# JuanJoZP/cfd-hemodynamic

Measured on AMD Instinct MI355X. Metric: time-steps/sec, dfg_1 ~1M DOF (stabilized_schur), higher is better.
Workload: dtype f64 (fp32 only in the AMG matrix values of the flexible preconditioner and in a read-only copy of the Krylov basis that Gram-Schmidt reads in solves of >= 20 iterations)

## Files before the change

### cfd_hemodynamic_amd/csrc/cfdh_api.cpp

```cpp
#include <algorithm>
#include <cmath>
#include <numeric>

#include <dlfcn.h>

#include "cfdh_internal.hpp"

std::string g_cfdh_last_error;

int cfdh_prepare_assembly(cfdh_ctx *c);

#define ENTER(c)                         \
  do {                                   \
    if (!(c)) return CFDH_E_ARG;         \
    (void)hipSetDevice((c)->device);     \
  } while (0)

extern "C" {

int cfdh_abi_version(void) { return CFDH_ABI_VERSION; }

const char *cfdh_last_error(const cfdh_ctx *c) { return c ? c->err.c_str() : g_cfdh_last_error.c_str(); }

int cfdh_default_options(cfdh_options *o) {
// ... 5 lines not shown
  o->pc_refresh = 0; o->remove_p_mean = 1; o->verbose = 0; o->pc_type = 1; o->cc_smooth_degree = 2;
  o->ksp_guess = getenv("CFDH_KSP_GUESS") ? atoi(getenv("CFDH_KSP_GUESS")) : 4;
  return 0;
}

static int create_ctx(cfdh_ctx **out, int device, int gdim, int etype, int64_t nv, int64_t nv_owned, int64_t nc, const int32_t *cells,
                      const double *coords, int64_t nfacets, const int32_t *facet_cells, const int32_t *facet_local,
                      const int32_t *facet_marker) {
  if (!out) return cfdh_fail(nullptr, CFDH_E_ARG, "null output pointer");
  *out = nullptr;
  if (gdim != 2 && gdim != 3) return cfdh_fail(nullptr, CFDH_E_ARG, "gdim must be 2 (P1 triangles) or 3 (P1 tetrahedra)");
  if (etype < 0 || etype > 3) return cfdh_fail(nullptr, CFDH_E_ARG, "unknown element type %d", etype);
  if (!cells || !coords || (nfacets > 0 && (!facet_cells || !facet_local)))
    return cfdh_fail(nullptr, CFDH_E_ARG, "null mesh array");
  int ndev = 0;
  if (hipGetDeviceCount(&ndev) != hipSuccess || ndev <= 0)
    return cfdh_fail(nullptr, CFDH_E_HIP, "no HIP device available: libcfdh has no CPU fallback");
  if (device < 0 || device >= ndev) return cfdh_fail(nullptr, CFDH_E_ARG, "device %d out of range (%d devices)", device, ndev);
  cfdh_ctx *c = new (std::nothrow) cfdh_ctx();
  if (!c) return cfdh_fail(nullptr, CFDH_E_NOMEM, "out of host memory");
  c->device = device;
  cfdh_default_options(&c->opt);
  { const char *e = getenv("CFDH_NO_GRAPH"); c->use_graph = !(e && e[0] == '1'); }
  if (c->use_graph && (getenv("ROCP_TOOL_LIBRARIES") || dlsym(RTLD_DEFAULT, "rocprofiler_configure"))) {
    int rt = 0;
    const char *ov = getenv("CFDH_GRAPH_UNDER_PROFILER");
    if (!(ov && ov[0] == '1') && hipRuntimeGetVersion(&rt) == hipSuccess && rt >= 70200000) c->use_graph = false;
  }
  memset(&c->last_stats, 0, sizeof c->last_stats);
  int rc = 0;
  do {
    if (hipSetDevice(device) != hipSuccess) { rc = cfdh_fail(nullptr, CFDH_E_HIP, "hipSetDevice(%d) failed", device); break; }
    if (hipStreamCreateWithFlags(&c->stream, hipStreamNonBlocking) != hipSuccess) { rc = cfdh_fail(nullptr, CFDH_E_HIP, "hipStreamCreate failed"); break; }
    rc = gdim == 3 ? k3_upload_quadrature(c) : k_upload_quadrature(c);
    if (rc) break;
    if (etype != 0) {
      rc = gdim == 3 ? kg3_upload_tables(c) : kg_upload_tables(c);
      if (rc) break;
      rc = gdim == 3 ? cfdh_build_mesh_gen3(c, etype, nv, nv_owned, nc, cells, coords, nfacets, facet_cells, facet_local, facet_marker)
                     : cfdh_build_mesh_gen(c, etype, nv, nv_owned, nc, cells, coords, nfacets, facet_cells, facet_local, facet_marker);
      break;
    }
    rc = gdim == 3 ? cfdh_build_mesh3(c, nv, nv_owned, nc, cells, coords, nfacets, facet_cells, facet_local, facet_marker)
                   : cfdh_build_mesh(c, nv, nv_owned, nc, cells, coords, nfacets, facet_cells, facet_local, facet_marker);
  } while (0);
  if (rc) {
// ... 15 lines not shown
                     int64_t nfacets, const int32_t *facet_cells, const int32_t *facet_local, const int32_t *facet_marker) {
  return create_ctx(out, device, gdim, elem, nn, nn, nc, cells, node_coords, nfacets, facet_cells, facet_local, facet_marker);
}

int cfdh_create_elem_part(cfdh_ctx **out, int device, int gdim, int elem, int64_t nn, int64_t nn_owned, int64_t nc, const int32_t *cells,
                          const double *node_coords, int64_t nfacets, const int32_t *facet_cells, const int32_t *facet_local, const int32_t *facet_marker) {
  return create_ctx(out, device, gdim, elem, nn, nn_owned, nc, cells, node_coords, nfacets, facet_cells, facet_local, facet_marker);
}

void cfdh_destroy(cfdh_ctx *c) {
  if (!c) return;
  (void)hipSetDevice(c->device);
  if (c->stream) (void)hipStreamSynchronize(c->stream);
  comm_finalize(c);
  c->hS.clear(); c->hL.clear(); c->hA.clear(); c->hLg.clear();
  for (hipEvent_t e : c->ev_pool) (void)hipEventDestroy(e);
  for (auto &e : c->pc_graphs) for (auto &x : e.exec) if (x) (void)hipGraphExecDestroy(x);
  if (c->h_pinned) (void)hipHostFree(c->h_pinned);
  if (c->h_stage) (void)hipHostFree(c->h_stage);
  if (c->ev_h) (void)hipEventDestroy(c->ev_h);
  if (c->h_big) (void)hipHostFree(c->h_big);
  if (c->h_ring) (void)hipHostFree(c->h_ring);
  for (hipEvent_t e : c->ev_ring) if (e) (void)hipEventDestroy(e);
  hipStream_t s = c->stream;
  delete c;
  if (s) (void)hipStreamDestroy(s);
}

int cfdh_set_params(cfdh_ctx *c, double dt, double rho, double mu, double mu_facet, const double f[3]) {
  ENTER(c);
  if (!(dt > 0) || !(rho > 0) || !(mu > 0)) return cfdh_fail(c, CFDH_E_ARG, "dt, rho, mu must be positive");
  const bool changed = !c->params_set || dt != c->dt || rho != c->rho || mu != c->mu;
  c->dt = dt; c->rho = rho; c->mu = mu; c->muf = mu_facet;
  c->f[0] = f ? f[0] : 0.0; c->f[1] = f ? f[1] : 0.0; c->f[2] = (f && c->dim == 3) ? f[2] : 0.0;
  c->params_set = true;
  if (changed) { c->mom_valid = false; c->pc_valid = false; }
  return 0;
}

int cfdh_set_options(cfdh_ctx *c, const cfdh_options *o) {
  if (!c || !o) return CFDH_E_ARG;
  if (o->ksp_restart < 1 || o->ksp_restart > 1000 || o->cheb_degree < 1 || o->cc_smooth_degree < 1 || !(o->cheb_ratio > 1) || o->amg_smooth_degree < 1 ||
      !(o->amg_smooth_ratio > 1) || o->amg_max_coarse < 8 || o->amg_max_coarse > 4000 || o->ksp_guess < 0 || o->ksp_guess > 8)
    return cfdh_fail(c, CFDH_E_ARG, "option out of range");
  const bool pc_changed = o->amg_theta != c->opt.amg_theta || o->amg_max_coarse != c->opt.amg_max_coarse ||
                          o->amg_smooth_ratio != c->opt.amg_smooth_ratio || o->pc_type != c->opt.pc_type ||
                          o->amg_smooth_degree != c->opt.amg_smooth_degree ||
                          o->schur_full != c->opt.schur_full;
// ... 682 lines not shown
```

### cfd_hemodynamic_amd/csrc/cfdh_internal.hpp

```cpp
#pragma once
#include <hip/hip_runtime.h>

#include <cstdint>
#include <cstdio>
#include <cstring>
#include <string>
#include <vector>

#include "cfdh.h"

#ifndef CFDH_MAX_INC
#define CFDH_MAX_INC 256
#endif
#ifndef CFDH_MAX_BV
#define CFDH_MAX_BV 192
#endif
#ifndef CFDH_MAX_BC
#define CFDH_MAX_BC 192
#endif
#ifndef CFDH_MAX_ROWS
#define CFDH_MAX_ROWS 128
#endif

#if defined(__HIPCC__)
// ... 215 lines not shown
  dbuf<double> kV, kZ, kw, kh;
  dbuf<float> kV32;
  bool krylov_fp32_ok = true;
  int guess_last_its[4] = {0, 0, 0, 0};
  dbuf<double> ky;

  dbuf<double> dinvA;
  double lmaxA = 0;
  dbuf<double> pu0, pu1, pu2, pr, pp0, pp1;
  dbuf<double> prand;
  dbuf<double> cheb_coef;
  struct PcGraph { const double *r; double *z; hipGraphExec_t exec[6]; };
  std::vector<PcGraph> pc_graphs;
  bool pc_graph_valid = false, capturing = false, use_graph = true;
  AmgHier hS;
  AmgHier hL;
  AmgHier hA;
  AmgLevel Hlev;
  dbuf<double> ccMl;
  dbuf<unsigned char> ccPbc;
  double cc_alpha = 0, cc_beta = 0;
  int up0_rows = 0;
  struct Epilogue { bool on = false, done = false; double alpha = 0, beta = 0; const double *zH = nullptr, *r = nullptr; const unsigned char *pbc = nullptr; double *out = nullptr; } epi;
  std::vector<double> h_Lval, h_Ml;
  dbuf<double> d_Lval, d_Ml;
  dbuf<double> amg_rand;
  double ms_pc_build_dev = 0;
  long long bc_version = 0;
  int gp_n = 0;
  CsrHost gp_L;
  bool gp_singular = false, gp_dirty = false;
  AmgHier hLg;
  dbuf<int> gp_l2g;
  dbuf<double> gp_rhs, gp_sol;
  bool ras = false;
  std::vector<int> h_gid;
  std::vector<int> h_g2l;
  dbuf<double> ras_b, ras_x;
  struct RasPlan {
    bool ready = false;
    int maxlen = 0;
    int nent = 0;
    dbuf<int> gptr, gcol, gsrc;
    dbuf<double> gval;
  } rasp;
  struct DistL0 {
// ... 97 lines not shown
int kg_assemble(cfdh_ctx *c, const double *xstate, int mode);
int kg_functional_partials(cfdh_ctx *c, int kind, int marker, int nb);
int kg_wss(cfdh_ctx *c, double *out);

int kg3_upload_tables(cfdh_ctx *c);
int cfdh_build_mesh_gen3(cfdh_ctx *c, int etype, int64_t nv, int64_t nv_owned, int64_t nc, const int32_t *cells, const double *coords, int64_t nfac,
                         const int32_t *fcell, const int32_t *flocal, const int32_t *fmarker);
int cfdh_gen3_element_stiffness(const cfdh_ctx *c, const int32_t *v, const double *X, double *K);
int cfdh_facet_nodes3(const cfdh_ctx *c, int f, int out[8]);
int kg3_assemble(cfdh_ctx *c, const double *xstate, int mode);
int kg3_functional_partials(cfdh_ctx *c, int kind, int marker, int nb);
int kg3_wss(cfdh_ctx *c, double *out);

void prof_begin(cfdh_ctx *c, int kind);
void prof_end(cfdh_ctx *c, int kind);
void prof_flush(cfdh_ctx *c);

int k_upload_quadrature(cfdh_ctx *c);
int k_halo_pack(cfdh_ctx *c, const double *vec);
int v_pointwise_mult(cfdh_ctx *c, int n, const double *a, const double *b, double *out);
int k_moments(cfdh_ctx *c);
int k_assemble(cfdh_ctx *c, const double *xstate, int mode);
int k_spmv_full(cfdh_ctx *c, const double *x, double *y);
int k_spmv_full_multi(cfdh_ctx *c, const double *X, double *Y, int ld, int nvec);
int k_spmv_block(cfdh_ctx *c, int blk, const double *x, double *y, const double *b, double alpha);
int k_spmv_block_ghost(cfdh_ctx *c, int blk, const double *xv, double *y, const double *b);
int k_extract_diag(cfdh_ctx *c);
int k_cheb_a00(cfdh_ctx *c, const double *b, double *x);
int k_cheb_a00_coeffs(cfdh_ctx *c);
int k_csr_spmv(cfdh_ctx *c, const CsrDev &A, const double *x, double *y, int mode, const double *b);
int k_csr_spmv_ncol(cfdh_ctx *c, const CsrDev &A, const double *x, double *y, int mode, const double *b, int ncol);
int k_amg_vcycle(cfdh_ctx *c, AmgHier &H, const double *b, double *x);
int k_level_smooth(cfdh_ctx *c, AmgLevel *L, const double *b, double *x, int degree);
bool k_cc_cheb2_scale(cfdh_ctx *c, AmgLevel *L, const double *b, double *x, const double *ml, double *y);
int k_cc_scale(cfdh_ctx *c, int n, const double *ml, const double *z, double *y);
int k_dl0_down(cfdh_ctx *c, const double *halo_vec);
int k_dl0_up(cfdh_ctx *c, double *out);
int k_ext_pack(cfdh_ctx *c, const double *vec, double *out);
int k_scatter_global(cfdh_ctx *c, int n, const int *l2g, const double *loc, double *glob);
int k_gather_global(cfdh_ctx *c, int n, const int *l2g, const double *glob, double *loc);
int k_cc_combine(cfdh_ctx *c, int n, double alpha, double beta, const double *t, const double *z, const double *r, const unsigned char *pbc, double *out, double *out2 = nullptr);
int k_nullspace_test(cfdh_ctx *c, double *nrm, double *absnrm);
int k_bc_scatter(cfdh_ctx *c, int n, int ncomp, const int *idx, const unsigned char *flag, const double *val, const double *mult);

int v_copy(cfdh_ctx *c, int n, const double *x, double *y);
int v_zero(cfdh_ctx *c, int n, double *y);
// ... 39 lines not shown
```

### cfd_hemodynamic_amd/csrc/cfdh_kernels.hip

```cpp
#include <hip/hip_runtime.h>

#include <cmath>

#include "cfdh_internal.hpp"
#include "cfdh_quad_tri.h"

#define TPB 256
#define NTLOAD(p) __builtin_nontemporal_load(p)

__constant__ double d_qw[CFDH_NQ];
__constant__ double d_ql[CFDH_NQ][3];

int k_upload_quadrature(cfdh_ctx *c) {
  HIPCHK(c, hipMemcpyToSymbol(HIP_SYMBOL(d_qw), CFDH_QW, sizeof(CFDH_QW)));
  HIPCHK(c, hipMemcpyToSymbol(HIP_SYMBOL(d_ql), CFDH_QL, sizeof(CFDH_QL)));
  return 0;
}

void prof_begin(cfdh_ctx *c, int kind) {
  if (!c->prof_on || c->capturing) return;
  if (c->ev_next + 2 > c->ev_pool.size()) {
    for (int i = 0; i < 64; i++) { hipEvent_t e; if (hipEventCreate(&e) != hipSuccess) return; c->ev_pool.push_back(e); }
  }
  cfdh_ctx::EvRec r;
// ... 731 lines not shown
  if (row < nvo) {
    const int ks = vptr[row], ke = vptr[row + 1];
    if (l == 0) bb = *(const double2 *)(bvec + 2 * (size_t)row);
    const int k0 = ks + l, k1 = k0 + 4;
    const bool h0 = k0 < ke, h1 = k1 < ke;
    const int q0 = h0 ? k0 : ks, q1 = h1 ? k1 : ks;
    const int w0 = vcol[q0], w1 = vcol[q1];
    const double2 c0 = *(const double2 *)(A + 2 * (size_t)q0), c1 = *(const double2 *)(A + 2 * (size_t)q1);
    const double x0 = (h0 && w0 < nvo) ? x[w0] : 0.0, x1 = (h1 && w1 < nvo) ? x[w1] : 0.0;
    a0 = c0.x * x0 + c1.x * x1;
    a1 = c0.y * x0 + c1.y * x1;
    for (int k = k1 + 4; k < ke; k += 4) {
      const int w = vcol[k];
      if (w >= nvo) continue;
      const double xp = x[w];
      const double2 cc = *(const double2 *)(A + 2 * (size_t)k);
      a0 += cc.x * xp; a1 += cc.y * xp;
    }
  }
  a0 = quad_sum(a0); a1 = quad_sum(a1);
  if (row < nvo && l == 0) *(double2 *)(y + 2 * (size_t)row) = make_double2(bb.x - a0, bb.y - a1);
}

template <int GB>
__global__ __launch_bounds__(TPB) void spmv_blk_ghost_kernel(int nvo, const int *__restrict__ vptr, const int *__restrict__ vcol,
                                                             const double *__restrict__ A, const double *__restrict__ xv,
                                                             double *__restrict__ y, const double *__restrict__ bvec) {
  const int gid = blockIdx.x * TPB + threadIdx.x;
  const int row = gid >> 3, l = gid & 7;
  double a0 = 0, a1 = 0;
  if (row < nvo) {
    const int ks = vptr[row], ke = vptr[row + 1];
    for (int k = ks + l; k < ke; k += 8) {
      const int w = vcol[k];
      const double2 cc = *(const double2 *)(A + 2 * (size_t)k);
      if (GB == 2) {
        const double xp = xv[poff(w, nvo)];
        a0 += cc.x * xp; a1 += cc.y * xp;
      } else {
        const int uo = uoff(w, nvo);
        a0 += cc.x * xv[uo] + cc.y * xv[uo + 1];
      }
    }
  }
  a0 = group8_sum(a0);
  if (GB == 2) a1 = group8_sum(a1);
// ... 583 lines not shown
    T gb[2], gc[2];
#pragma unroll
    for (int q = 0; q < 2; q++) {
      if (kb + 8 * q < keB) gb[q] = b[cb[q]];
      if (kc + 8 * q < keC) gc[q] = xc[cc[q]];
    }
#pragma unroll
    for (int q = 0; q < 2; q++) {
      if (kb + 8 * q < keB) a = vfma(vb[q], gb[q], a);
      if (kc + 8 * q < keC) a = vfma(vc[q], gc[q], a);
    }
    for (int k = kb + 16; k < keB; k += 8) a = vfma(vlB[k], b[clB[k]], a);
    for (int k = kc + 16; k < keC; k += 8) a = vfma(vlC[k], xc[clC[k]], a);
  }
  a = g8(a);
  if (row < n && l == 0) x[row] = epbc ? epi_apply(a, row, ea, eb, ezH, er, epbc) : a;
}
template <typename T, bool WIDE>
__global__ __launch_bounds__(TPB) void fused_up_sell_kernel(int n, const int *__restrict__ spB, const int *__restrict__ scB,
                                                            const float *__restrict__ svB, const T *__restrict__ b,
                                                            const int *__restrict__ spC, const int *__restrict__ scC,
                                                            const float *__restrict__ svC, const T *__restrict__ xc,
                                                            T *__restrict__ x, double ea, double eb, const double *__restrict__ ezH,
                                                            const double *__restrict__ er, const unsigned char *__restrict__ epbc) {
  const int row = blockIdx.x * TPB + threadIdx.x;
  if (row >= n) return;
  const int sl = __builtin_amdgcn_readfirstlane(row >> 6), lane = row & 63;
  T a = vzero((const T *)nullptr);
  double e_zh = 0.0, e_r = 0.0;
  unsigned e_f = 0;
  if (epbc) { e_f = epbc[row]; e_zh = ezH[row]; e_r = er[row]; }
  constexpr int MW = sizeof(T) > 8 ? 8 : 10;
  const int pB = spB[sl], wB = (spB[sl + 1] - pB) >> 6;
  int pC = 0, wC = 0;
  if (spC) { pC = spC[sl]; wC = (spC[sl + 1] - pC) >> 6; }
  const int wmax = wB > wC ? wB : wC;
  for (int k0 = 0; k0 < (WIDE ? wmax : 1); k0 += MW) {
    int cB[MW], cC[MW];
    float vB[MW], vC[MW];
#pragma unroll
    for (int k = 0; k < MW; k++) if (k0 + k < wB) { const int p = pB + (k0 + k) * 64 + lane; cB[k] = NTLOAD(scB + p); vB[k] = NTLOAD(svB + p); }
#pragma unroll
    for (int k = 0; k < MW; k++) if (k0 + k < wC) { const int p = pC + (k0 + k) * 64 + lane; cC[k] = NTLOAD(scC + p); vC[k] = NTLOAD(svC + p); }
    T gB[MW], gC[MW];
#pragma unroll
    for (int k = 0; k < MW; k++) if (k0 + k < wB) gB[k] = b[cB[k]];
#pragma unroll
    for (int k = 0; k < MW; k++) if (k0 + k < wC) gC[k] = xc[cC[k]];
#pragma unroll
    for (int k = 0; k < MW; k++) if (k0 + k < wB) a = vfma((double)vB[k], gB[k], a);
#pragma unroll
    for (int k = 0; k < MW; k++) if (k0 + k < wC) a = vfma((double)vC[k], gC[k], a);
  }
  if (!WIDE) {
    for (int k = MW; k < wB; k++) { const int p = pB + k * 64 + lane; a = vfma((double)svB[p], b[scB[p]], a); }
    for (int k = MW; k < wC; k++) { const int p = pC + k * 64 + lane; a = vfma((double)svC[p], xc[scC[p]], a); }
// ... 17 lines not shown
    for (int q = 0; q < 12; q++) { const int j = l + 64 * q; if (j < nc) { dv[q] = Dr[j]; bv[q] = bc[j]; } }
#pragma unroll
    for (int q = 0; q < 12; q++) { const int j = l + 64 * q; if (j < nc) a = vfma((double)dv[q], bv[q], a); }
    for (int j = l + 768; j < nc; j += 64) a = vfma((double)Dr[j], bc[j], a);
  }
  a = wsum(a);
  if (row < n && l == 0) x[row] = a;
}

template <typename VT, typename T>
static void launch_down(cfdh_ctx *c, const CsrDev &G, const VT *val, const T *x, T *y) {
  const long long avg = G.n > 0 ? (G.nnz + G.n - 1) / G.n : 1;
  const int lpr = avg > 96 ? 64 : (avg > 48 ? 32 : (avg > 20 ? 16 : 8));
  dim3 block(TPB), grid((unsigned)(((long long)G.n * lpr + TPB - 1) / TPB));
  if (lpr == 64) hipLaunchKernelGGL((fused_down_kernel<64, VT, T>), grid, block, 0, c->stream, G.n, G.rowptr.p, G.col.p, val, x, y);
  else if (lpr == 32) hipLaunchKernelGGL((fused_down_kernel<32, VT, T>), grid, block, 0, c->stream, G.n, G.rowptr.p, G.col.p, val, x, y);
  else if (lpr == 16) hipLaunchKernelGGL((fused_down_kernel<16, VT, T>), grid, block, 0, c->stream, G.n, G.rowptr.p, G.col.p, val, x, y);
  else hipLaunchKernelGGL((fused_down_kernel<8, VT, T>), grid, block, 0, c->stream, G.n, G.rowptr.p, G.col.p, val, x, y);
}

template <typename T>
static int amg_cycle_fused(cfdh_ctx *c, AmgHier &H, const T *b, T *x, int prof, int l0 = 0) {
  const int nl = (int)H.lev.size();
  for (int l = l0; l + 1 < nl; l++) {
    AmgLevel *L = H.lev[l], *N = H.lev[l + 1];
    const T *src = l == l0 ? b : (const T *)L->b.p;
    if (prof && l == 0) prof_begin(c, prof + 4);
    if (L->fine) launch_down<float, T>(c, L->G, L->G.valf.p, src, (T *)N->b.p);
    else launch_down<double, T>(c, L->G, L->G.val.p, src, (T *)N->b.p);
    if (prof && l == 0) prof_end(c, prof + 4);
  }
  int l = nl - 1;
  {
    AmgLevel *L = H.lev[l];
    const T *bl = l == l0 ? b : (const T *)L->b.p;
    T *xl = l == l0 ? x : (T *)L->x.p;
    if (nl - 2 >= l0 && H.lev[nl - 2]->Dn > 0) {
      AmgLevel *U = H.lev[nl - 2];
      const T *bu = nl - 2 == l0 ? b : (const T *)U->b.p;
      T *xu = nl - 2 == l0 ? x : (T *)U->x.p;
      const int un = (nl - 2 == 0 && c->up0_rows > 0 && c->up0_rows < U->n) ? c->up0_rows : U->n;
      hipLaunchKernelGGL((fused_up_dense_kernel<T>), dim3((unsigned)((64ll * un + TPB - 1) / TPB)), dim3(TPB), 0, c->stream, un,
                         U->Sb.rowptr.p, U->Sb.col.p, U->Sb.val.p, bu, U->D.p, U->Dn, bl, xu);
      l = nl - 3;
    } else {
      if (H.coarse_n > 0)
        hipLaunchKernelGGL((dense_mv_kernel<T>), dim3(H.coarse_n), dim3(64), 0, c->stream, H.coarse_n, H.coarse_inv.p, bl, xl);
      else if (L->sell)
        hipLaunchKernelGGL((fused_up_sell_kernel<T, true>), dim3((unsigned)((L->n + TPB - 1) / TPB)), dim3(TPB), 0, c->stream, L->n,
                           L->Sb.sptr.p, L->Sb.scol.p, L->Sb.sval.p, bl, (const int *)nullptr, (const int *)nullptr,
                           (const float *)nullptr, (const T *)nullptr, xl, 0.0, 0.0, (const double *)nullptr, (const double *)nullptr,
                           (const unsigned char *)nullptr);
      else
        hipLaunchKernelGGL((fused_up_csr_kernel<T>), dim3((unsigned)((8ll * L->n + TPB - 1) / TPB)), dim3(TPB), 0, c->stream, L->n,
                           L->Sb.rowptr.p, L->Sb.col.p, L->Sb.val.p, bl, (const int *)nullptr, (const int *)nullptr,
                           (const double *)nullptr, (const T *)nullptr, xl, 0.0, 0.0, (const double *)nullptr, (const double *)nullptr,
                           (const unsigned char *)nullptr);
      l = nl - 2;
    }
  }
  for (; l >= l0; l--) {
    AmgLevel *L = H.lev[l], *N = H.lev[l + 1];
    const T *bl = l == l0 ? b : (const T *)L->b.p;
    T *xl = l == l0 ? x : (T *)L->x.p;
    const bool epi = l == 0 && c->epi.on && sizeof(T) == sizeof(double);
    const double ea = epi ? c->epi.alpha : 0.0, eb = epi ? c->epi.beta : 0.0;
    const double *ezH = epi ? c->epi.zH : nullptr, *er = epi ? c->epi.r : nullptr;
    const unsigned char *epbc = epi ? c->epi.pbc : nullptr;
    if (epi) { xl = (T *)c->epi.out; c->epi.done = true; }
    const int nrow = (l == 0 && c->up0_rows > 0 && c->up0_rows < L->n) ? c->up0_rows : L->n;
    if (prof && l == 0) prof_begin(c, prof);
    if (L->sell && L->Sb.sell_maxw <= 14 && L->Sc.sell_maxw <= 14)
      hipLaunchKernelGGL((fused_up_sell_kernel<T, false>), dim3((unsigned)((nrow + TPB - 1) / TPB)), dim3(TPB), 0, c->stream, nrow,
                         L->Sb.sptr.p, L->Sb.scol.p, L->Sb.sval.p, bl, L->Sc.sptr.p, L->Sc.scol.p, L->Sc.sval.p, (const T *)N->x.p, xl,
                         ea, eb, ezH, er, epbc);
    else if (L->sell)
      hipLaunchKernelGGL((fused_up_sell_kernel<T, true>), dim3((unsigned)((nrow + TPB - 1) / TPB)), dim3(TPB), 0, c->stream, nrow,
                         L->Sb.sptr.p, L->Sb.scol.p, L->Sb.sval.p, bl, L->Sc.sptr.p, L->Sc.scol.p, L->Sc.sval.p, (const T *)N->x.p, xl,
                         ea, eb, ezH, er, epbc);
    else
      hipLaunchKernelGGL((fused_up_csr_kernel<T>), dim3((unsigned)((8ll * nrow + TPB - 1) / TPB)), dim3(TPB), 0, c->stream, nrow,
                         L->Sb.rowptr.p, L->Sb.col.p, L->Sb.val.p, bl, L->Sc.rowptr.p, L->Sc.col.p, L->Sc.val.p, (const T *)N->x.p, xl,
                         ea, eb, ezH, er, epbc);
    if (prof && l == 0) prof_end(c, prof);
  }
  HIPCHK(c, hipGetLastError());
  return 0;
}

static int amg_cycle_cheb(cfdh_ctx *c, AmgHier &H, size_t lev, const double *b, double *x, bool prof) {
  AmgLevel *L = H.lev[lev];
  if (lev + 1 == H.lev.size()) {
    if (H.coarse_n > 0) {
      hipLaunchKernelGGL((dense_mv_kernel<double>), dim3(H.coarse_n), dim3(64), 0, c->stream, H.coarse_n, H.coarse_inv.p, b, x);
      HIPCHK(c, hipGetLastError());
      return 0;
    }
    return level_cheb(c, L, b, x, true, c->opt.amg_smooth_degree > 2 ? c->opt.amg_smooth_degree : 2, false);
  }
  AmgLevel *N = H.lev[lev + 1];
  const int deg = c->opt.amg_smooth_degree;
  CHK(level_cheb(c, L, b, x, true, deg, prof && lev == 0));
  CHK(k_csr_spmv(c, L->A, x, L->r.p, 1, b));
  CHK(k_csr_spmv(c, L->R, L->r.p, N->b.p, 0, nullptr));
  CHK(amg_cycle_cheb(c, H, lev + 1, N->b.p, N->x.p, prof));
  CHK(k_csr_spmv(c, L->P, N->x.p, x, 2, nullptr));
  CHK(level_cheb(c, L, b, x, false, deg, prof && lev == 0));
// ... 900 lines not shown
```

### cfd_hemodynamic_amd/csrc/cfdh_solver.cpp

```cpp
#include <algorithm>
#include <chrono>
#include <cmath>

#include "cfdh_internal.hpp"

int cfdh_host_threads();

static double wall_ms() {
  using namespace std::chrono;
  return duration<double, std::milli>(steady_clock::now().time_since_epoch()).count();
}

int cfdh_download_blocks(cfdh_ctx *c, std::vector<double> &a00, std::vector<double> &a01, std::vector<double> &a10,
                         std::vector<double> &a11) {
  const size_t nz = (size_t)c->nnzv, d = (size_t)c->dim;
  a00.resize(d * d * nz); a01.resize(d * nz); a10.resize(d * nz); a11.resize(nz);
  HIPCHK(c, hipMemcpyAsync(a00.data(), c->A00.p, sizeof(double) * d * d * nz, hipMemcpyDeviceToHost, c->stream));
  HIPCHK(c, hipMemcpyAsync(a01.data(), c->A01.p, sizeof(double) * d * nz, hipMemcpyDeviceToHost, c->stream));
  HIPCHK(c, hipMemcpyAsync(a10.data(), c->A10.p, sizeof(double) * d * nz, hipMemcpyDeviceToHost, c->stream));
  HIPCHK(c, hipMemcpyAsync(a11.data(), c->A11.p, sizeof(double) * nz, hipMemcpyDeviceToHost, c->stream));
  HIPCHK(c, hipStreamSynchronize(c->stream));
  return 0;
}

// ... 407 lines not shown
    CHK(k_spmv_block(c, 1, v, w, nullptr, 0));
    CHK(v_pointwise_mult(c, nu, w, c->dinvA.p, w));
    CHK(v_norm_to_dev(c, nu, w, c->red_out.p + 4));
    CHK(v_scale_inv_dev(c, nu, w, c->red_out.p + 4, v));
  }
  HIPCHK(c, hipMemcpyAsync(c->h_pinned, c->red_out.p + 4, sizeof(double), hipMemcpyDeviceToHost, c->stream));
  HIPCHK(c, hipStreamSynchronize(c->stream));
  lam = c->h_pinned[0];
  if (!(lam > 0) || !std::isfinite(lam)) return cfdh_fail(c, CFDH_E_DIVERGED, "non-finite spectral estimate of D^-1 A00 (NaN in the Jacobian?)");
  c->lmaxA = 1.15 * lam;
  CHK(k_cheb_a00_coeffs(c));
  if (refresh_amg || !c->pc_valid) {
    c->pc_graph_valid = false;
    CsrHost S;
    CHK(build_schur_host(c, S));
    bool any_pbc = false;
    for (int i = 0; i < c->nvo; i++) any_pbc |= (c->h_bcflag[i] & (1u << c->dim)) != 0;
    CHK(cfdh_amg_setup(c, c->hS, S, c->singular != 0 || !any_pbc, 1));
    c->pc_valid = true;
    c->pc_its_ref = 0;
    c->steps_since_refresh = 0;
    c->last_stats.pc_refreshes++;
    c->n_pc_builds++;
  }
  return 0;
}

static bool ras_ghost_rhs() {
  static const bool on = !(getenv("CFDH_RAS_GHOST_RHS") && getenv("CFDH_RAS_GHOST_RHS")[0] == '0');
  return on;
}

static int pc_stage(cfdh_ctx *c, const double *r, double *z, int stage) {
  const int nvo = c->nvo, nu = c->dim * nvo;
  const double *ru = r, *rp = r + nu;
  double *zu = z, *zp = z + nu;
  const bool multi = c->nranks > 1;
  const bool global_p = c->gp_n > 0 && multi;
  if (c->opt.pc_type == 1) {
    const bool upper = c->opt.schur_full == 2;
    const bool dist = global_p && c->dl0.on;
    int ls = stage;
    if (dist) ls = stage <= 1 ? stage : (stage == 2 ? 10 : stage - 1);
    switch (ls) {
      case 0:
        if (upper) return 0;
// ... 24 lines not shown
        if (dist) {
          CHK(k_dl0_up(c, c->pu2.p));
        } else if (global_p) {
          if (c->gp_allgather) CHK(k_gather_global(c, c->gp_n, c->gp_src_idx.p, c->gp_recvbuf.p, c->gp_rhs.p));
          CHK(k_amg_vcycle(c, c->hLg, c->gp_rhs.p, c->gp_sol.p));
          CHK(k_gather_global(c, nvo, c->gp_l2g.p, c->gp_sol.p, c->pu2.p));
        } else {
          static const int lcycles = getenv("CFDH_L_CYCLES") ? atoi(getenv("CFDH_L_CYCLES")) : 1;
          if (lcycles > 1 && c->hL.lev.size() >= 1 && c->hL.lev[0]->A.val.p) {
            AmgLevel *L0 = c->hL.lev[0];
            CHK(k_amg_vcycle(c, c->hL, c->pu1.p, c->pu2.p));
            for (int cyc = 1; cyc < lcycles; cyc++) {
              CHK(k_csr_spmv(c, L0->A, c->pu2.p, L0->r.p, 1, c->pu1.p));
              CHK(k_amg_vcycle(c, c->hL, L0->r.p, L0->d0.p));
              CHK(v_axpy(c, nvo, 1.0, L0->d0.p, c->pu2.p));
            }
            CHK(k_cc_combine(c, nvo, c->cc_alpha, c->cc_beta, c->pu2.p, c->pp1.p, upper ? rp : c->pp0.p, c->ccPbc.p, zp));
            if (multi && c->opt.schur_full) CHK(v_copy(c, nvo, zp, c->pcw.p + nu));
            return 0;
          }
          c->epi.on = true; c->epi.done = false;
          c->epi.alpha = c->cc_alpha; c->epi.beta = c->cc_beta; c->epi.zH = c->pp1.p; c->epi.r = upper ? rp : c->pp0.p;
          c->epi.pbc = c->ccPbc.p; c->epi.out = zp;
          const int rc = k_amg_vcycle(c, c->hL, c->pu1.p, c->pu2.p);
          c->epi.on = false;
          CHK(rc);
        }
        if (c->epi.done) {
          c->epi.done = false;
          if (multi && c->opt.schur_full) CHK(v_copy(c, nvo, zp, c->pcw.p + nu));
        } else {
          CHK(k_cc_combine(c, nvo, c->cc_alpha, c->cc_beta, c->pu2.p, c->pp1.p, upper ? rp : c->pp0.p, c->ccPbc.p, zp,
                           (multi && c->opt.schur_full) ? c->pcw.p + nu : nullptr));
        }
        return 0;
      case 3:
        if (c->opt.schur_full) {
          if (multi) CHK(k_spmv_block_ghost(c, 2, c->pcw.p, c->ras ? c->pcw.p : c->pu0.p, ru));
          else CHK(k_spmv_block(c, 2, zp, c->pu0.p, ru, 0));
          if (multi && c->ras) {
            if (!ras_ghost_rhs()) CHK(v_zero(c, c->NL - c->NO, c->pcw.p + c->NO));
          }
          else {
            CHK(k_amg_vcycle(c, c->hA, c->pu0.p, zu));
            static const int acycles = getenv("CFDH_A_CYCLES") ? atoi(getenv("CFDH_A_CYCLES")) : 1;
            if (acycles > 1 && !multi && c->hA.lev[0]->A.val.p) {
              AmgLevel *L0 = c->hA.lev[0];
              for (int cyc = 1; cyc < acycles; cyc++) {
                CHK(k_csr_spmv_ncol(c, L0->A, zu, L0->r.p, 1, c->pu0.p, c->dim));
                CHK(k_amg_vcycle(c, c->hA, L0->r.p, L0->d0.p));
                CHK(v_axpy(c, nu, 1.0, L0->d0.p, zu));
              }
            }
          }
        } else {
          CHK(v_copy(c, nu, multi ? c->pcw.p : c->pu0.p, zu));
        }
        return 0;
      case 4:
        if (multi && c->ras && c->opt.schur_full) {
          CHK(k_ext_pack(c, c->pcw.p, c->ras_b.p));
          if (c->hA.fused && c->opt.amg_smooth_degree == 1 && c->hA.lev.size() >= 2) {
            c->up0_rows = nvo;
            const int rc = k_amg_vcycle(c, c->hA, c->ras_b.p, zu);
            c->up0_rows = 0;
            CHK(rc);
          } else {
// ... 23 lines not shown
  if (c->nranks <= 1 || c->opt.pc_type != 1) return 0;
  const bool dist = c->gp_n > 0 && c->dl0.on;
  int ls = stage;
  if (dist) ls = stage <= 1 ? stage : (stage == 2 ? 10 : stage - 1);
  switch (ls) {
    case 0: return c->opt.schur_full == 2 ? 0 : comm_halo(c, c->pcw.p);
    case 1:
      if (c->gp_n <= 0) return 0;
      if (dist) return c->dl0.ghost_rhs ? comm_halo(c, c->pcw.p) : 0;
      if (c->gp_allgather) return comm_allgather_dev(c, c->gp_sendbuf.p, c->gp_recvbuf.p, c->gp_maxcnt);
      return comm_allreduce_dev(c, c->gp_rhs.p, c->gp_n, 0);
    case 10: return comm_allreduce_dev(c, c->hLg.lev[1]->b.p, c->dl0.n1, 0);
    case 2: return c->opt.schur_full ? comm_halo(c, c->pcw.p) : 0;
    case 3: return (c->ras && c->opt.schur_full && ras_ghost_rhs()) ? comm_halo(c, c->pcw.p) : 0;
    default: return 0;
  }
}

int cfdh_pc_apply(cfdh_ctx *c, const double *r, double *z) {
  const int nvo = c->nvo;
  const bool graph = c->use_graph && !c->prof_on;
  const bool multi = c->nranks > 1 && c->opt.pc_type == 1;
  if (multi && !c->pcw.p) { HIPCHK(c, c->pcw.alloc(c->NL)); HIPCHK(c, c->pcw.zero(c->stream)); }
  if (!graph) {
    for (int st = 0; st < 6; st++) { CHK(pc_stage(c, r, z, st)); CHK(pc_exchange(c, st)); }
  } else {
    if (!c->pc_graph_valid) {
      for (auto &e : c->pc_graphs) for (auto &x : e.exec) if (x) (void)hipGraphExecDestroy(x);
      c->pc_graphs.clear();
      c->pc_graph_valid = true;
    }
    cfdh_ctx::PcGraph *pg = nullptr;
    for (auto &e : c->pc_graphs) if (e.r == r && e.z == z) { pg = &e; break; }
    if (!pg) {
      cfdh_ctx::PcGraph ng{r, z, {nullptr, nullptr, nullptr, nullptr, nullptr, nullptr}};
      for (int gidx = 0; gidx < (multi ? 6 : 1); gidx++) {
        hipGraph_t g = nullptr;
        HIPCHK(c, hipStreamBeginCapture(c->stream, hipStreamCaptureModeThreadLocal));
        c->capturing = true;
        int rc = 0;
        if (multi) rc = pc_stage(c, r, z, gidx);
        else for (int st = 0; st < 6 && !rc; st++) rc = pc_stage(c, r, z, st);
        c->capturing = false;
        hipError_t e = hipStreamEndCapture(c->stream, &g);
        if (rc) return rc;
        if (e != hipSuccess || !g) return cfdh_fail(c, CFDH_E_HIP, "hipStreamEndCapture: %s", hipGetErrorString(e));
// ... 250 lines not shown
    first = false;
    std::fill(g.begin(), g.end(), 0.0);
    g[0] = beta;
    static const int refine_env = getenv("CFDH_GS_REFINE_FROM") ? atoi(getenv("CFDH_GS_REFINE_FROM")) : -1;
    static const int lag_env = getenv("CFDH_KSP_LAG") ? atoi(getenv("CFDH_KSP_LAG")) : cfdh_ctx::KRING - 3;
    const int refine_from = refine_env >= 0 ? refine_env : (c->gs_refine_long ? 24 : (1 << 30));
    const int lagmax = (o.ksp_rtol < 1e-7 || c->prof_on) ? 0 : std::max(0, std::min(lag_env, cfdh_ctx::KRING - 3));
    const int its_base = its;
    const int maxl = std::min(m, o.ksp_max_it - its_base);
    int j = 0;
    int jl = 0;
    const int e_its = (gslot >= 0 && gslot < cfdh_ctx::GUESS_NEWTON) ? c->guess_last_its[gslot] : 0;
    int need = std::max(1, std::min(e_its - its - 2, 3));
    double res_hist[4] = {beta, 0, 0, 0};
    int nhist = 1;
    bool done = false;
    double *s_dev = hd + 2 * (m + 2) + 1;
    const size_t rs = c->h_ring_stride;
    auto launch = [&](int jj) -> int {
      double *vj = V + (size_t)jj * ld, *zj = Z + (size_t)jj * ld, *vn = V + (size_t)(jj + 1) * ld;
      double *slot = c->h_ring_dev + (size_t)(jj % cfdh_ctx::KRING) * rs;
      CHK(cfdh_pc_apply(c, vj, zj));
      CHK(comm_halo(c, zj));
      CHK(k_spmv_full(c, zj, w));
      if (use32) {
        CHK(v_multidot32(c, n, V32, (int)ld32, jj + 1, w, hd, slot));
        CHK(v_gs_update32(c, n, V32, (int)ld32, jj + 1, hd, w, vn, V32 + (size_t)(jj + 1) * ld32, s_dev, slot + (jj + 2)));
        HIPCHK(c, hipEventRecord(c->ev_ring[jj % cfdh_ctx::KRING], c->stream));
      } else {
        CHK(v_multidot(c, n, V, (int)ld, jj + 1, w, hd, true, slot));
        HIPCHK(c, hipEventRecord(c->ev_ring[jj % cfdh_ctx::KRING], c->stream));
        CHK(v_gs_update_normalize(c, n, V, (int)ld, jj + 1, hd, w, vn, s_dev));
      }
      return 0;
    };
    while (!done && reason == 0) {
      const bool sync_now = lagmax == 0 || j >= refine_from;
      const int ahead = sync_now ? 1 : std::max(1, std::min(need - (need >= 4 ? 1 : 0), lagmax + 1));
      while (jl < maxl && jl - j < ahead) { CHK(launch(jl)); jl++; }
      if (jl == j) break;
      int upto = jl;
      if (!sync_now && jl - j > 1 && jl < maxl && need > jl - j) upto = jl - 1;
      c->n_host_sync++;
      HIPCHK(c, hipEventSynchronize(c->ev_ring[(upto - 1) % cfdh_ctx::KRING]));
      for (; j < upto && !done; ) {
        const double *hs = c->h_ring + (size_t)(j % cfdh_ctx::KRING) * rs;
        double *vn = V + (size_t)(j + 1) * ld;
        double ww = hs[j + 1], hh2 = 0.0;
        for (int i = 0; i <= j; i++) { hh[i] = hs[i]; hh2 += hh[i] * hh[i]; }
        double nrm2 = use32 ? hs[j + 2] * hs[j + 2] : ww - hh2;
        static const double eta2_env = getenv("CFDH_GS_ETA2") ? atof(getenv("CFDH_GS_ETA2")) : 1e-6;
        const double eta2 = (o.ksp_rtol < 1e-7 || j >= refine_from) ? 0.5 : eta2_env;
        const bool refine = !(nrm2 > eta2 * ww);
        double hnorm;
        if (refine) {
          if (jl > j + 1) { c->n_krylov_discarded += jl - (j + 1); jl = j + 1; }
          CHK(v_multidot(c, n, V, (int)ld, j + 1, vn, hd + (m + 2), true));
          CHK(v_multiaxpy(c, n, V, (int)ld, j + 1, hd + (m + 2), vn));
          if (use32) CHK(v_norm_to_dev(c, n, vn, hd + 2 * (m + 2)));
          HIPCHK(c, hipMemcpyAsync(c->h_pinned, hd + (m + 2), sizeof(double) * (m + 4), hipMemcpyDeviceToHost, c->stream));
          c->n_host_sync++;
          HIPCHK(c, hipStreamSynchronize(c->stream));
          const double s = use32 ? hs[j + 2] : ((nrm2 > 0.0 && nrm2 <= ww) ? std::sqrt(nrm2) : std::sqrt(ww));
          double h22 = 0.0;
          for (int i = 0; i <= j; i++) { hh[i] += s * c->h_pinned[i]; h22 += c->h_pinned[i] * c->h_pinned[i]; }
          double vnorm;
          if (use32) vnorm = c->h_pinned[m + 2];
          else {
            const double d2 = c->h_pinned[j + 1] - h22;
            vnorm = d2 > 0.0 ? std::sqrt(d2) : 0.0;
          }
          hnorm = s * vnorm;
          if (use32) { CHK(v_scale_inv_dev(c, n, vn, hd + 2 * (m + 2), vn)); CHK(v_store32(c, n, vn, V32 + (size_t)(j + 1) * ld32)); }
          else CHK(v_scale(c, n, vnorm > 0.0 ? 1.0 / vnorm : 0.0, vn));
        } else {
          hnorm = std::sqrt(nrm2);
        }
        double *Hj = &H[(size_t)j * (m + 1)];
        for (int i = 0; i <= j; i++) Hj[i] = hh[i];
// ... 208 lines not shown
```

Measured before the change: 421.6.

## Reuse pressure-column SpMV from Schur stage in Krylov matvec; optional second-stream AMG overlap

The Schur-complement preconditioner stage now computes the pressure-column products (A01·p and A11·p) as a by-product of its residual kernel and stores them in a scratch buffer. The outer Krylov matvec then only evaluates the velocity-column part and adds the stored result, so the pressure-column SpMV is no longer done twice. An opt-in mode (iter_overlap>=2) goes further: it runs those pressure columns and the first AMG up-sweep B-part on a second stream, joined by events. The change also adds a fix that resets the sync window after Gram-Schmidt refinement, and it is only enabled for serial 2D P1 stabilized_schur configurations.

```diff
diff --git a/cfd_hemodynamic_amd/csrc/cfdh_api.cpp b/cfd_hemodynamic_amd/csrc/cfdh_api.cpp
--- a/cfd_hemodynamic_amd/csrc/cfdh_api.cpp
+++ b/cfd_hemodynamic_amd/csrc/cfdh_api.cpp
@@ -51,6 +51,7 @@
   c->device = device;
   cfdh_default_options(&c->opt);
   { const char *e = getenv("CFDH_NO_GRAPH"); c->use_graph = !(e && e[0] == '1'); }
+  { const char *e = getenv("CFDH_ITER_OVERLAP"); c->iter_overlap = (e && *e) ? atoi(e) : 1; }
   if (c->use_graph && (getenv("ROCP_TOOL_LIBRARIES") || dlsym(RTLD_DEFAULT, "rocprofiler_configure"))) {
     int rt = 0;
     const char *ov = getenv("CFDH_GRAPH_UNDER_PROFILER");
@@ -112,8 +113,10 @@
   if (c->h_big) (void)hipHostFree(c->h_big);
   if (c->h_ring) (void)hipHostFree(c->h_ring);
   for (hipEvent_t e : c->ev_ring) if (e) (void)hipEventDestroy(e);
-  hipStream_t s = c->stream;
+  for (hipEvent_t e : {c->ev_fork, c->ev_join, c->ev_join_p}) if (e) (void)hipEventDestroy(e);
+  hipStream_t s = c->stream, s2 = c->stream2;
   delete c;
+  if (s2) (void)hipStreamDestroy(s2);
   if (s) (void)hipStreamDestroy(s);
 }
 
diff --git a/cfd_hemodynamic_amd/csrc/cfdh_internal.hpp b/cfd_hemodynamic_amd/csrc/cfdh_internal.hpp
--- a/cfd_hemodynamic_amd/csrc/cfdh_internal.hpp
+++ b/cfd_hemodynamic_amd/csrc/cfdh_internal.hpp
@@ -261,6 +261,11 @@
   double cc_alpha = 0, cc_beta = 0;
   int up0_rows = 0;
   struct Epilogue { bool on = false, done = false; double alpha = 0, beta = 0; const double *zH = nullptr, *r = nullptr; const unsigned char *pbc = nullptr; double *out = nullptr; } epi;
+  int iter_overlap = 1;
+  bool split_up = false;
+  hipStream_t stream2 = nullptr;
+  hipEvent_t ev_fork = nullptr, ev_join = nullptr, ev_join_p = nullptr;
+  dbuf<double> jzp;
   std::vector<double> h_Lval, h_Ml;
   dbuf<double> d_Lval, d_Ml;
   dbuf<double> amg_rand;
@@ -404,6 +409,9 @@
 int k_moments(cfdh_ctx *c);
 int k_assemble(cfdh_ctx *c, const double *xstate, int mode);
 int k_spmv_full(cfdh_ctx *c, const double *x, double *y);
+int k_spmv_pcols_side(cfdh_ctx *c, const double *xp, double *ap);
+int k_spmv_a01_resid_pcols(cfdh_ctx *c, const double *xp, double *y, const double *b, double *ap);
+int k_spmv_jz_finish(cfdh_ctx *c, const double *x, const double *ap, double *y);
 int k_spmv_full_multi(cfdh_ctx *c, const double *X, double *Y, int ld, int nvec);
 int k_spmv_block(cfdh_ctx *c, int blk, const double *x, double *y, const double *b, double alpha);
 int k_spmv_block_ghost(cfdh_ctx *c, int blk, const double *xv, double *y, const double *b);
diff --git a/cfd_hemodynamic_amd/csrc/cfdh_kernels.hip b/cfd_hemodynamic_amd/csrc/cfdh_kernels.hip
--- a/cfd_hemodynamic_amd/csrc/cfdh_kernels.hip
+++ b/cfd_hemodynamic_amd/csrc/cfdh_kernels.hip
@@ -777,6 +777,111 @@
   if (row < nvo && l == 0) *(double2 *)(y + 2 * (size_t)row) = make_double2(bb.x - a0, bb.y - a1);
 }
 
+__global__ __launch_bounds__(TPB) void spmv_pcols_kernel(int nvo, const int *__restrict__ vptr, const int *__restrict__ vcol,
+                                                         const double *__restrict__ A01, const double *__restrict__ A11,
+                                                         const double *__restrict__ xp, double *__restrict__ ap) {
+  const int gid = blockIdx.x * TPB + threadIdx.x;
+  const int row = gid >> 3, l = gid & 7;
+  double a0 = 0, a1 = 0, a2 = 0;
+  if (row < nvo) {
+    const int ks = vptr[row], ke = vptr[row + 1];
+    for (int k = ks + l; k < ke; k += 8) {
+      const double x = xp[vcol[k]];
+      const double2 c01 = *(const double2 *)(A01 + 2 * (size_t)k);
+      a0 += c01.x * x; a1 += c01.y * x; a2 += A11[k] * x;
+    }
+  }
+  a0 = group8_sum(a0); a1 = group8_sum(a1); a2 = group8_sum(a2);
+  if (row < nvo && l == 0) {
+    *(double2 *)(ap + 2 * (size_t)row) = make_double2(a0, a1);
+    ap[2 * (size_t)nvo + row] = a2;
+  }
+}
+__global__ __launch_bounds__(TPB) void spmv_jz_finish_kernel(int nvo, const int *__restrict__ vptr, const int *__restrict__ vcol,
+                                                             const double *__restrict__ A00, const double *__restrict__ A10,
+                                                             const double *__restrict__ x, const double *__restrict__ ap,
+                                                             double *__restrict__ y) {
+  const int gid = blockIdx.x * TPB + threadIdx.x;
+  const int row = gid >> 3, l = gid & 7;
+  double a0 = 0, a1 = 0, a2 = 0;
+  double2 pu = make_double2(0.0, 0.0);
+  double pp = 0.0;
+  if (row < nvo) {
+    if (l == 0) { pu = *(const double2 *)(ap + 2 * (size_t)row); pp = ap[2 * (size_t)nvo + row]; }
+    const int ks = vptr[row], ke = vptr[row + 1];
+    for (int k = ks + l; k < ke; k += 8) {
+      const double2 xu = *(const double2 *)(x + 2 * (size_t)vcol[k]);
+      const double2 b0 = *(const double2 *)(A00 + 4 * (size_t)k), b1 = *(const double2 *)(A00 + 4 * (size_t)k + 2);
+      const double2 c10 = *(const double2 *)(A10 + 2 * (size_t)k);
+      a0 += b0.x * xu.x + b0.y * xu.y;
+      a1 += b1.x * xu.x + b1.y * xu.y;
+      a2 += c10.x * xu.x + c10.y * xu.y;
+    }
+  }
+  a0 = group8_sum(a0); a1 = group8_sum(a1); a2 = group8_sum(a2);
+  if (row < nvo && l == 0) {
+    *(double2 *)(y + 2 * (size_t)row) = make_double2(a0 + pu.x, a1 + pu.y);
+    y[2 * (size_t)nvo + row] = a2 + pp;
+  }
+}
+__global__ __launch_bounds__(TPB) void spmv_a01_resid_pcols_kernel(int nvo, const int *__restrict__ vptr, const int *__restrict__ vcol,
+                                                                   const double *__restrict__ A01, const double *__restrict__ A11,
+                                                                   const double *__restrict__ x, double *__restrict__ y,
+                                                                   const double *__restrict__ bvec, double *__restrict__ ap) {
+  const int gid = blockIdx.x * TPB + threadIdx.x;
+  const int row = gid >> 2, l = gid & 3;
+  double a0 = 0, a1 = 0, a2 = 0;
+  double2 bb = make_double2(0.0, 0.0);
+  if (row < nvo) {
+    const int ks = vptr[row], ke = vptr[row + 1];
+    if (l == 0) bb = *(const double2 *)(bvec + 2 * (size_t)row);
+    const int k0 = ks + l, k1 = k0 + 4;
+    const bool h0 = k0 < ke, h1 = k1 < ke;
+    const int q0 = h0 ? k0 : ks, q1 = h1 ? k1 : ks;
+    const int w0 = vcol[q0], w1 = vcol[q1];
+    const double2 c0 = *(const double2 *)(A01 + 2 * (size_t)q0), c1 = *(const double2 *)(A01 + 2 * (size_t)q1);
+    const double d0 = A11[q0], d1 = A11[q1];
+    const double x0 = (h0 && w0 < nvo) ? x[w0] : 0.0, x1 = (h1 && w1 < nvo) ? x[w1] : 0.0;
+    a0 = c0.x * x0 + c1.x * x1;
+    a1 = c0.y * x0 + c1.y * x1;
+    a2 = d0 * x0 + d1 * x1;
+    for (int k = k1 + 4; k < ke; k += 4) {
+      const int w = vcol[k];
+      if (w >= nvo) continue;
+      const double xp = x[w];
+      const double2 cc = *(const double2 *)(A01 + 2 * (size_t)k);
+      a0 += cc.x * xp; a1 += cc.y * xp; a2 += A11[k] * xp;
+    }
+  }
+  a0 = quad_sum(a0); a1 = quad_sum(a1); a2 = quad_sum(a2);
+  if (row < nvo && l == 0) {
+    *(double2 *)(y + 2 * (size_t)row) = make_double2(bb.x - a0, bb.y - a1);
+    *(double2 *)(ap + 2 * (size_t)row) = make_double2(a0, a1);
+    ap[2 * (size_t)nvo + row] = a2;
+  }
+}
+int k_spmv_a01_resid_pcols(cfdh_ctx *c, const double *xp, double *y, const double *b, double *ap) {
+  const long long n4 = 4ll * c->nvo;
+  hipLaunchKernelGGL(spmv_a01_resid_pcols_kernel, dim3((unsigned)((n4 + TPB - 1) / TPB)), dim3(TPB), 0, c->stream, c->nvo, c->vptr.p,
+                     c->vcol.p, c->A01.p, c->A11.p, xp, y, b, ap);
+  HIPCHK(c, hipGetLastError());
+  return 0;
+}
+int k_spmv_pcols_side(cfdh_ctx *c, const double *xp, double *ap) {
+  const long long nthreads = 8ll * c->nvo;
+  hipLaunchKernelGGL(spmv_pcols_kernel, dim3((unsigned)((nthreads + TPB - 1) / TPB)), dim3(TPB), 0, c->stream2, c->nvo, c->vptr.p,
+                     c->vcol.p, c->A01.p, c->A11.p, xp, ap);
+  HIPCHK(c, hipGetLastError());
+  return 0;
+}
+int k_spmv_jz_finish(cfdh_ctx *c, const double *x, const double *ap, double *y) {
+  const long long nthreads = 8ll * c->nvo;
+  hipLaunchKernelGGL(spmv_jz_finish_kernel, dim3((unsigned)((nthreads + TPB - 1) / TPB)), dim3(TPB), 0, c->stream, c->nvo, c->vptr.p,
+                     c->vcol.p, c->A00.p, c->A10.p, x, ap, y);
+  HIPCHK(c, hipGetLastError());
+  return 0;
+}
+
 template <int GB>
 __global__ __launch_bounds__(TPB) void spmv_blk_ghost_kernel(int nvo, const int *__restrict__ vptr, const int *__restrict__ vcol,
                                                              const double *__restrict__ A, const double *__restrict__ xv,
@@ -1406,16 +1511,18 @@
                                                             const int *__restrict__ spC, const int *__restrict__ scC,
                                                             const float *__restrict__ svC, const T *__restrict__ xc,
                                                             T *__restrict__ x, double ea, double eb, const double *__restrict__ ezH,
-                                                            const double *__restrict__ er, const unsigned char *__restrict__ epbc) {
+                                                            const double *__restrict__ er, const unsigned char *__restrict__ epbc,
+                                                            const T *__restrict__ tb) {
   const int row = blockIdx.x * TPB + threadIdx.x;
   if (row >= n) return;
   const int sl = __builtin_amdgcn_readfirstlane(row >> 6), lane = row & 63;
-  T a = vzero((const T *)nullptr);
+  T a = tb ? tb[row] : vzero((const T *)nullptr);
   double e_zh = 0.0, e_r = 0.0;
   unsigned e_f = 0;
   if (epbc) { e_f = epbc[row]; e_zh = ezH[row]; e_r = er[row]; }
   constexpr int MW = sizeof(T) > 8 ? 8 : 10;
-  const int pB = spB[sl], wB = (spB[sl + 1] - pB) >> 6;
+  int pB = 0, wB = 0;
+  if (!tb) { pB = spB[sl]; wB = (spB[sl + 1] - pB) >> 6; }
   int pC = 0, wC = 0;
   if (spC) { pC = spC[sl]; wC = (spC[sl + 1] - pC) >> 6; }
   const int wmax = wB > wC ? wB : wC;
@@ -1479,6 +1586,26 @@
 template <typename T>
 static int amg_cycle_fused(cfdh_ctx *c, AmgHier &H, const T *b, T *x, int prof, int l0 = 0) {
   const int nl = (int)H.lev.size();
+  AmgLevel *F = H.lev[l0];
+  const bool split = c->split_up && l0 == 0 && F->sell && F->Dn == 0 && c->up0_rows == 0 && c->stream2 &&
+                     F->d1.n >= (size_t)F->n * (sizeof(T) / sizeof(double));
+  const bool wide0 = !(F->Sb.sell_maxw <= 14 && F->Sc.sell_maxw <= 14);
+  T *tb = split ? (T *)F->d1.p : nullptr;
+  if (split) {
+    HIPCHK(c, hipEventRecord(c->ev_fork, c->stream));
+    HIPCHK(c, hipStreamWaitEvent(c->stream2, c->ev_fork, 0));
+    const dim3 gr((unsigned)((F->n + TPB - 1) / TPB)), bl(TPB);
+    if (wide0)
+      hipLaunchKernelGGL((fused_up_sell_kernel<T, true>), gr, bl, 0, c->stream2, F->n, F->Sb.sptr.p, F->Sb.scol.p, F->Sb.sval.p, b,
+                         (const int *)nullptr, (const int *)nullptr, (const float *)nullptr, (const T *)nullptr, tb, 0.0, 0.0,
+                         (const double *)nullptr, (const double *)nullptr, (const unsigned char *)nullptr, (const T *)nullptr);
+    else
+      hipLaunchKernelGGL((fused_up_sell_kernel<T, false>), gr, bl, 0, c->stream2, F->n, F->Sb.sptr.p, F->Sb.scol.p, F->Sb.sval.p, b,
+                         (const int *)nullptr, (const int *)nullptr, (const float *)nullptr, (const T *)nullptr, tb, 0.0, 0.0,
+                         (const double *)nullptr, (const double *)nullptr, (const unsigned char *)nullptr, (const T *)nullptr);
+    HIPCHK(c, hipGetLastError());
+    HIPCHK(c, hipEventRecord(c->ev_join, c->stream2));
+  }
   for (int l = l0; l + 1 < nl; l++) {
     AmgLevel *L = H.lev[l], *N = H.lev[l + 1];
     const T *src = l == l0 ? b : (const T *)L->b.p;
@@ -1507,7 +1634,7 @@
         hipLaunchKernelGGL((fused_up_sell_kernel<T, true>), dim3((unsigned)((L->n + TPB - 1) / TPB)), dim3(TPB), 0, c->stream, L->n,
                            L->Sb.sptr.p, L->Sb.scol.p, L->Sb.sval.p, bl, (const int *)nullptr, (const int *)nullptr,
                            (const float *)nullptr, (const T *)nullptr, xl, 0.0, 0.0, (const double *)nullptr, (const double *)nullptr,
-                           (const unsigned char *)nullptr);
+                           (const unsigned char *)nullptr, (const T *)nullptr);
       else
         hipLaunchKernelGGL((fused_up_csr_kernel<T>), dim3((unsigned)((8ll * L->n + TPB - 1) / TPB)), dim3(TPB), 0, c->stream, L->n,
                            L->Sb.rowptr.p, L->Sb.col.p, L->Sb.val.p, bl, (const int *)nullptr, (const int *)nullptr,
@@ -1526,20 +1653,22 @@
     const unsigned char *epbc = epi ? c->epi.pbc : nullptr;
     if (epi) { xl = (T *)c->epi.out; c->epi.done = true; }
     const int nrow = (l == 0 && c->up0_rows > 0 && c->up0_rows < L->n) ? c->up0_rows : L->n;
-    if (prof && l == 0) prof_begin(c, prof);
+    const T *tl = (split && l == l0) ? tb : nullptr;
+    if (tl) HIPCHK(c, hipStreamWaitEvent(c->stream, c->ev_join, 0));
+    if (prof && l == 0 && !tl) prof_begin(c, prof);
     if (L->sell && L->Sb.sell_maxw <= 14 && L->Sc.sell_maxw <= 14)
       hipLaunchKernelGGL((fused_up_sell_kernel<T, false>), dim3((unsigned)((nrow + TPB - 1) / TPB)), dim3(TPB), 0, c->stream, nrow,
                          L->Sb.sptr.p, L->Sb.scol.p, L->Sb.sval.p, bl, L->Sc.sptr.p, L->Sc.scol.p, L->Sc.sval.p, (const T *)N->x.p, xl,
-                         ea, eb, ezH, er, epbc);
+                         ea, eb, ezH, er, epbc, tl);
     else if (L->sell)
       hipLaunchKernelGGL((fused_up_sell_kernel<T, true>), dim3((unsigned)((nrow + TPB - 1) / TPB)), dim3(TPB), 0, c->stream, nrow,
                          L->Sb.sptr.p, L->Sb.scol.p, L->Sb.sval.p, bl, L->Sc.sptr.p, L->Sc.scol.p, L->Sc.sval.p, (const T *)N->x.p, xl,
-                         ea, eb, ezH, er, epbc);
+                         ea, eb, ezH, er, epbc, tl);
     else
       hipLaunchKernelGGL((fused_up_csr_kernel<T>), dim3((unsigned)((8ll * nrow + TPB - 1) / TPB)), dim3(TPB), 0, c->stream, nrow,
                          L->Sb.rowptr.p, L->Sb.col.p, L->Sb.val.p, bl, L->Sc.rowptr.p, L->Sc.col.p, L->Sc.val.p, (const T *)N->x.p, xl,
                          ea, eb, ezH, er, epbc);
-    if (prof && l == 0) prof_end(c, prof);
+    if (prof && l == 0 && !tl) prof_end(c, prof);
   }
   HIPCHK(c, hipGetLastError());
   return 0;
diff --git a/cfd_hemodynamic_amd/csrc/cfdh_solver.cpp b/cfd_hemodynamic_amd/csrc/cfdh_solver.cpp
--- a/cfd_hemodynamic_amd/csrc/cfdh_solver.cpp
+++ b/cfd_hemodynamic_amd/csrc/cfdh_solver.cpp
@@ -453,6 +453,23 @@
     c->steps_since_refresh = 0;
     c->last_stats.pc_refreshes++;
     c->n_pc_builds++;
+  }
+  return 0;
+}
+
+static bool overlap_cfg(const cfdh_ctx *c) {
+  return c->nranks <= 1 && c->dim == 2 && c->etype == 0 && !c->gen && c->opt.pc_type == 1 && c->opt.schur_full == 2;
+}
+static bool overlap_pc(const cfdh_ctx *c) { return c->iter_overlap >= 2 && overlap_cfg(c); }
+static bool overlap_jz(const cfdh_ctx *c) { return c->iter_overlap >= 1 && overlap_cfg(c) && !c->singular; }
+static int ensure_overlap(cfdh_ctx *c) {
+  if (overlap_jz(c) && !c->jzp.p) HIPCHK(c, c->jzp.alloc(c->NL));
+  if (!overlap_pc(c)) return 0;
+  if (!c->stream2) {
+    HIPCHK(c, hipStreamCreateWithFlags(&c->stream2, hipStreamNonBlocking));
+    HIPCHK(c, hipEventCreateWithFlags(&c->ev_fork, hipEventDisableTiming));
+    HIPCHK(c, hipEventCreateWithFlags(&c->ev_join, hipEventDisableTiming));
+    HIPCHK(c, hipEventCreateWithFlags(&c->ev_join_p, hipEventDisableTiming));
   }
   return 0;
 }
@@ -523,8 +540,10 @@
           c->epi.on = true; c->epi.done = false;
           c->epi.alpha = c->cc_alpha; c->epi.beta = c->cc_beta; c->epi.zH = c->pp1.p; c->epi.r = upper ? rp : c->pp0.p;
           c->epi.pbc = c->ccPbc.p; c->epi.out = zp;
+          c->split_up = overlap_pc(c);
           const int rc = k_amg_vcycle(c, c->hL, c->pu1.p, c->pu2.p);
           c->epi.on = false;
+          c->split_up = false;
           CHK(rc);
         }
         if (c->epi.done) {
@@ -538,12 +557,26 @@
       case 3:
         if (c->opt.schur_full) {
           if (multi) CHK(k_spmv_block_ghost(c, 2, c->pcw.p, c->ras ? c->pcw.p : c->pu0.p, ru));
-          else CHK(k_spmv_block(c, 2, zp, c->pu0.p, ru, 0));
+          else if (overlap_jz(c) && !overlap_pc(c)) {
+            CHK(k_spmv_a01_resid_pcols(c, zp, c->pu0.p, ru, c->jzp.p));
+          } else {
+            if (overlap_jz(c)) {
+              HIPCHK(c, hipEventRecord(c->ev_fork, c->stream));
+              HIPCHK(c, hipStreamWaitEvent(c->stream2, c->ev_fork, 0));
+              CHK(k_spmv_pcols_side(c, zp, c->jzp.p));
+              HIPCHK(c, hipEventRecord(c->ev_join_p, c->stream2));
+            }
+            CHK(k_spmv_block(c, 2, zp, c->pu0.p, ru, 0));
+          }
           if (multi && c->ras) {
             if (!ras_ghost_rhs()) CHK(v_zero(c, c->NL - c->NO, c->pcw.p + c->NO));
           }
           else {
-            CHK(k_amg_vcycle(c, c->hA, c->pu0.p, zu));
+            c->split_up = overlap_pc(c);
+            const int rc = k_amg_vcycle(c, c->hA, c->pu0.p, zu);
+            c->split_up = false;
+            CHK(rc);
+            if (overlap_jz(c) && overlap_pc(c)) HIPCHK(c, hipStreamWaitEvent(c->stream, c->ev_join_p, 0));
             static const int acycles = getenv("CFDH_A_CYCLES") ? atoi(getenv("CFDH_A_CYCLES")) : 1;
             if (acycles > 1 && !multi && c->hA.lev[0]->A.val.p) {
               AmgLevel *L0 = c->hA.lev[0];
@@ -613,6 +646,7 @@
   const bool graph = c->use_graph && !c->prof_on;
   const bool multi = c->nranks > 1 && c->opt.pc_type == 1;
   if (multi && !c->pcw.p) { HIPCHK(c, c->pcw.alloc(c->NL)); HIPCHK(c, c->pcw.zero(c->stream)); }
+  CHK(ensure_overlap(c));
   if (!graph) {
     for (int st = 0; st < 6; st++) { CHK(pc_stage(c, r, z, st)); CHK(pc_exchange(c, st)); }
   } else {
@@ -909,7 +943,8 @@
       double *slot = c->h_ring_dev + (size_t)(jj % cfdh_ctx::KRING) * rs;
       CHK(cfdh_pc_apply(c, vj, zj));
       CHK(comm_halo(c, zj));
-      CHK(k_spmv_full(c, zj, w));
+      if (overlap_jz(c)) CHK(k_spmv_jz_finish(c, zj, c->jzp.p, w));
+      else CHK(k_spmv_full(c, zj, w));
       if (use32) {
         CHK(v_multidot32(c, n, V32, (int)ld32, jj + 1, w, hd, slot));
         CHK(v_gs_update32(c, n, V32, (int)ld32, jj + 1, hd, w, vn, V32 + (size_t)(jj + 1) * ld32, s_dev, slot + (jj + 2)));
@@ -942,6 +977,7 @@
         double hnorm;
         if (refine) {
           if (jl > j + 1) { c->n_krylov_discarded += jl - (j + 1); jl = j + 1; }
+          upto = j + 1;
           CHK(v_multidot(c, n, V, (int)ld, j + 1, vn, hd + (m + 2), true));
           CHK(v_multiaxpy(c, n, V, (int)ld, j + 1, hd + (m + 2), vn));
           if (use32) CHK(v_norm_to_dev(c, n, vn, hd + 2 * (m + 2)));
```

Result: no change. 423.3 (median of 6 runs) (+0.4%).
